# Ntropy86/review-recommender

Measured on AMD Instinct MI355X. Metric: queries/sec at top-k=100 (hybrid alpha=0.5), higher is better.
Workload: dtype f32; 1 GPU; hybrid BM25+dense alpha=0.5 top-k=100 pool=150, 10000000 products x 384 fp32, BM25 ~40 tokens/doc vocab 200000 (327073593 postings on rank 0, 11164874 postings per query), batches of 256 queries; query_sets=4, docs=10000000, docs_per_gpu=10000000, batch=256, k=100, pool=150, parallelism=single GPU: no collective

## Files before the change

include/rr_hip.h:

```cpp
#ifndef RR_HIP_H
#define RR_HIP_H

#include <stdint.h>

#ifdef __cplusplus
extern "C" {
#endif

#define RR_OK            0
#define RR_E_INVALID    -1
#define RR_E_HIP        -2
#define RR_E_NOMEM      -3
#define RR_E_STATE      -4

#define RR_DTYPE_F32     0
#define RR_DTYPE_BF16    1

#define RR_MAX_POOL   2048
#define RR_MAX_BATCH  1024
#define RR_MAX_QTERMS   64

typedef struct rr_index rr_index;
typedef struct rr_bm25  rr_bm25;

// ... 79 lines not shown
    int32_t cand_per_rank;
    int32_t bm25_f64;
    int64_t cand_rank_stride_bytes;
} rr_fuse_params;

int rr_fuse_topk_dev(rr_index* ix, const rr_fuse_params* p, int32_t n_queries,
                     const int64_t* d_rows, const float* d_dense, const float* d_bm25,
                     const double* d_n_reviews, const double* d_avg_stars, const double* d_log1p_n,
                     const float* d_rerank, const float* d_best, const float* d_gate,
                     int64_t* d_out_rows, double* d_out_cols, int32_t* d_out_order, void* stream);
int rr_fuse_topk(rr_index* ix, const rr_fuse_params* p, int32_t n_queries,
                 const int64_t* h_rows, const float* h_dense, const float* h_bm25,
                 const double* h_n_reviews, const double* h_avg_stars, const double* h_log1p_n,
                 const float* h_rerank, const float* h_best, const float* h_gate,
                 int64_t* h_out_rows, double* h_out_cols, int32_t* h_out_order);
int rr_index_gather_meta_dev(rr_index* ix, const int64_t* d_rows, int64_t n,
                             double* d_n_reviews, double* d_avg_stars, double* d_log1p_n,
                             void* stream);

#define RR_COPY_MAX_SEGS 4
typedef struct rr_copy_seg {
    void* dst;
    const void* src;
    int64_t row_bytes, rows, dst_pitch, src_pitch;
} rr_copy_seg;
int rr_copy_segments_dev(const rr_copy_seg* segs, int32_t n_segs, int32_t device, void* stream);


typedef struct rr_reviews rr_reviews;
int rr_reviews_create(const float* h_emb, int64_t n_reviews, int32_t dim, int64_t n_products,
// ... 81 lines not shown
```

review-recommender_amd/_lib.py:

```python
from __future__ import annotations

import ctypes as C
import os
import threading

from .build import DEBUG_BUILD_ID, BUILD_ID, DEBUG_LIB_PATH, LIB_PATH, library_digest

c_i32, c_i64, c_f32, c_f64, c_vp = C.c_int32, C.c_int64, C.c_float, C.c_double, C.c_void_p
P = C.POINTER


class CopySeg(C.Structure):
    _fields_ = [("dst", C.c_void_p), ("src", C.c_void_p), ("row_bytes", C.c_int64), ("rows", C.c_int64),
                ("dst_pitch", C.c_int64), ("src_pitch", C.c_int64)]


class FuseParams(C.Structure):
    _fields_ = [("w_dense", c_f64), ("w_bm25", c_f64), ("w_rerank", c_f64),
                ("w_prior", c_f64), ("w_best", c_f64), ("prior_C", c_f64),
                ("min_reviews", c_i32), ("trust_sat", c_i32), ("apply_trust", c_i32),
                ("rerank_active", c_i32), ("rerank_k", c_i32), ("k", c_i32),
                ("n_candidates", c_i32), ("pool", c_i32), ("cand_per_rank", c_i32),
                ("bm25_f64", c_i32), ("cand_rank_stride_bytes", c_i64)]

# ... 38 lines not shown
    "rr_bm25_create": (C.c_int, [c_i32, c_i64, c_i64, c_i64, c_vp, c_vp, c_vp, c_vp, c_vp,
                                 c_vp, c_vp, c_vp, c_f64, c_f64, c_f64, c_i64, P(c_vp)]),
    "rr_bm25_create_dev": (C.c_int, [c_i32, c_i64, c_i64, c_i64, c_vp, c_vp, c_vp, c_vp, c_vp,
                                     c_vp, c_vp, c_vp, c_f64, c_f64, c_f64, c_i64, P(c_vp)]),
    "rr_bm25_destroy": (C.c_int, [c_vp]),
    "rr_bm25_get_scores": (C.c_int, [c_vp, c_vp, c_i32, c_vp]),
    "rr_bm25_scores_at": (C.c_int, [c_vp, c_vp, c_vp, c_i32, c_vp, c_i32, c_i32, c_vp]),
    "rr_bm25_scores_at_dev": (C.c_int, [c_vp, c_vp, c_vp, c_i32, c_vp, c_i32, c_i32, c_vp, c_vp]),
    "rr_bm25_build": (C.c_int, [c_i32, c_i32, c_vp, c_i64, c_vp, c_i64, c_i64, c_vp, c_i64, c_i64, c_i64,
                                c_f64, c_f64, c_i64, c_vp, P(c_vp)]),
    "rr_bm25_build_stats": (C.c_int, [c_vp, c_vp, c_vp]),
    "rr_bm25_set_idf": (C.c_int, [c_vp, c_vp, c_f64]),
    "rr_bm25_copy_csr": (C.c_int, [c_vp] + [c_vp] * 7),
    "rr_fuse_topk_dev": (C.c_int, [c_vp, P(FuseParams), c_i32] + [c_vp] * 9 + [c_vp] * 3 + [c_vp]),
    "rr_fuse_topk": (C.c_int, [c_vp, P(FuseParams), c_i32] + [c_vp] * 9 + [c_vp] * 3),
    "rr_index_gather_meta_dev": (C.c_int, [c_vp, c_vp, c_i64, c_vp, c_vp, c_vp, c_vp]),
    "rr_copy_segments_dev": (C.c_int, [c_vp, c_i32, c_i32, c_vp]),
    "rr_index_matrix_changed": (C.c_int, [c_vp]),
    "rr_reviews_create": (C.c_int, [c_vp, c_i64, c_i32, c_i64, c_vp, c_vp, c_i32, c_f32, P(c_vp)]),
    "rr_reviews_destroy": (C.c_int, [c_vp]),
    "rr_reviews_best_dev": (C.c_int, [c_vp, c_vp, c_i32, c_vp, c_i32, c_i64, c_i32, c_vp, c_vp, c_vp]),
    "rr_reviews_best_cut_dev": (C.c_int, [c_vp, c_vp, c_i32, c_vp, c_i32, c_i64, c_i64, c_vp, c_vp, c_vp]),
    "rr_ce_create": (C.c_int, [c_i32, P(CEConfig), P(c_vp), c_i32, P(c_vp)]),
    "rr_ce_destroy": (C.c_int, [c_vp]),
    "rr_ce_forward_dev": (C.c_int, [c_vp, c_vp, c_vp, c_vp, c_vp, c_i32, c_i64, c_i32, c_i32, c_vp, c_vp]),
    "rr_ce_last_forward_ms": (C.c_int, [c_vp, P(c_f32)]),
    "rr_ce_range_status": (C.c_int, [c_vp, P(C.c_int32)]),
    "rr_ce_set_wide_range": (C.c_int, [c_vp, C.c_int32]),
    "rr_wp_create": (C.c_int, [c_i32, c_vp, c_vp, c_i32, c_i32, c_i32, c_i32, c_i32, P(c_vp)]),
    "rr_wp_create_utf8": (C.c_int, [c_i32, c_vp, c_vp, c_i32, c_i32, c_i32, c_i32, c_i32, c_vp, c_i32, c_vp, c_i32, c_vp, c_i32,
# ... 85 lines not shown
```

review-recommender_amd/csrc/rr_bm25.hip:

```cpp
#include "rr_common.h"

#define RR_SLICE 4096
#define RR_AT_CANDS 64

struct rr_bm25_view {
    const int64_t* post_indptr;
    const int32_t* post_docs;
    const int32_t* post_tf;
    const int64_t* doc_indptr;
    const int32_t* doc_terms;
    const int32_t* doc_tf;
    const int32_t* doc_len;
    const double* idf;
    double avgdl, k1, b;
    int64_t n_docs, n_terms, row_offset;
};

__device__ __forceinline__ double rr_bm25_term(double idf, int tf, int dl, double avgdl, double k1,
                                               double b) {
    const double f = (double)tf;
    const double one_minus_b = 1.0 - b;
    const double norm = one_minus_b + (b * (double)dl) / avgdl;
    return idf * ((f * (k1 + 1.0)) / (f + k1 * norm));
}

__device__ __forceinline__ int64_t rr_lower_bound(const int32_t* __restrict__ a, int64_t lo,
                                                  int64_t hi, int32_t key) {
    while (lo < hi) {
        const int64_t mid = lo + ((hi - lo) >> 1);
        if (a[mid] < key) lo = mid + 1; else hi = mid;
    }
    return lo;
}

__device__ __forceinline__ int64_t rr_lower_bound_wave(const int32_t* __restrict__ a, int64_t lo, int64_t hi, int32_t key) {
    const int lane = threadIdx.x & 63;
    while (hi - lo > 64) {
        const int64_t stride = (hi - lo + 63) >> 6;
        const int64_t at = lo + lane * stride;
        const bool below = at < hi && a[at] < key;
        const int c = __popcll(__ballot(below));
        if (c == 0) return lo;
        const int64_t nlo = lo + (int64_t)(c - 1) * stride + 1, nhi = lo + (int64_t)c * stride;
        lo = nlo;
        hi = nhi < hi ? nhi : hi;
    }
    const bool below = lo + lane < hi && a[lo + lane] < key;
    return lo + __popcll(__ballot(below));
// ... 46 lines not shown
                    const int32_t dd = v.post_docs[p];
                    acc[dd - d0] += rr_bm25_term(idf, v.post_tf[p], v.doc_len[dd], v.avgdl, v.k1, v.b);
                }
            }
            __syncthreads();
        }
    }
    __syncthreads();
    const bool write = touched || dirty[blockIdx.x];
    if (write)
        for (int64_t i = tid; i < d1 - d0; i += 256) out[d0 + i] = acc[i];
    if (tid == 0) dirty[blockIdx.x] = (unsigned char)touched;
}

template <int MODE>
__global__ __launch_bounds__(256) void rr_bm25_at(rr_bm25_view v, const int32_t* __restrict__ term_ids,
                                                  const int32_t* __restrict__ term_off,
                                                  const int64_t* __restrict__ rows, int pool,
                                                  float* __restrict__ out) {
    __shared__ double contrib[RR_AT_CANDS][RR_MAX_QTERMS + 1];
    const int tid = threadIdx.x;
    const int q = blockIdx.y;
    const int c0 = blockIdx.x * RR_AT_CANDS;
    const int t0 = term_off[q];
    const int nt = term_off[q + 1] - t0;
    const int nc = pool - c0 < RR_AT_CANDS ? pool - c0 : RR_AT_CANDS;
    double sum = 0.0;

    for (int jb = 0; jb < nt; jb += RR_MAX_QTERMS) {
        const int nj = nt - jb < RR_MAX_QTERMS ? nt - jb : RR_MAX_QTERMS;
        for (int i = tid; i < nc * nj; i += 256) {
            const int c = i / nj, j = i % nj;
            const int64_t d = rows[(int64_t)q * pool + c0 + c] - v.row_offset;
            const int32_t t = term_ids[t0 + jb + j];
            double val = 0.0;
            if (d >= 0 && d < v.n_docs && t >= 0 && t < v.n_terms) {
                int tf = 0;
                if (MODE == 0) {
                    const int64_t s = v.doc_indptr[d], e = v.doc_indptr[d + 1];
                    const int64_t p = rr_lower_bound(v.doc_terms, s, e, t);
                    if (p < e && v.doc_terms[p] == t) tf = v.doc_tf[p];
                } else {
                    const int64_t s = v.post_indptr[t], e = v.post_indptr[t + 1];
                    const int64_t p = rr_lower_bound(v.post_docs, s, e, (int32_t)d);
                    if (p < e && v.post_docs[p] == (int32_t)d) tf = v.post_tf[p];
                }
                if (tf > 0) val = rr_bm25_term(v.idf[t], tf, v.doc_len[d], v.avgdl, v.k1, v.b);
            }
            contrib[c][j] = val;
        }
        __syncthreads();
        if (tid < nc)
            for (int j = 0; j < nj; ++j) sum += contrib[tid][j];
        __syncthreads();
    }
    if (tid < nc) out[(int64_t)q * pool + c0 + tid] = (float)sum;
}

template <typename T>
static int rr_upload(T** dst, const T* src, size_t n) {
    *dst = nullptr;
    RR_HIP_TRY(hipMalloc((void**)dst, sizeof(T) * (n ? n : 1)));
    if (n) RR_HIP_TRY(hipMemcpy(*dst, src, sizeof(T) * n, hipMemcpyHostToDevice));
    return RR_OK;
}

static rr_bm25_view rr_view(const rr_bm25* bm) {
    rr_bm25_view v;
    v.post_indptr = bm->d_post_indptr; v.post_docs = bm->d_post_docs; v.post_tf = bm->d_post_tf;
    v.doc_indptr = bm->d_doc_indptr; v.doc_terms = bm->d_doc_terms; v.doc_tf = bm->d_doc_tf;
    v.doc_len = bm->d_doc_len; v.idf = bm->d_idf;
    v.avgdl = bm->avgdl; v.k1 = bm->k1; v.b = bm->b;
    v.n_docs = bm->n_docs; v.n_terms = bm->n_terms; v.row_offset = bm->row_offset;
    return v;
}

extern "C" int rr_bm25_create(int32_t device, int64_t n_docs, int64_t n_terms, int64_t nnz,
                              const int64_t* post_indptr, const int32_t* post_docs,
                              const int32_t* post_tf, const int64_t* doc_indptr,
                              const int32_t* doc_terms, const int32_t* doc_tf,
                              const int32_t* doc_len, const double* idf, double avgdl, double k1,
                              double b, int64_t row_offset, rr_bm25** out) {
    RR_REQUIRE(out, "rr_bm25_create: NULL out");
    *out = nullptr;
    RR_REQUIRE(n_docs >= 1 && n_docs < (1ll << 31), "rr_bm25_create: n_docs %lld out of range",
               (long long)n_docs);
    RR_REQUIRE(n_terms >= 0 && n_terms < (1ll << 31) && nnz >= 0, "rr_bm25_create: bad sizes");
    RR_REQUIRE(post_indptr && doc_indptr && doc_len && (nnz == 0 || (post_docs && post_tf && doc_terms && doc_tf)) &&
                   (n_terms == 0 || idf),
// ... 181 lines not shown
```

review-recommender_amd/csrc/rr_fuse.hip:

```cpp
#include "rr_common.h"

#define RR_FUSE_THREADS 256
#define RR_FUSE_MAXCAND RR_MAX_CANDIDATES

struct rr_fuse_dev_params {
    rr_fuse_params p;
    double log1p_sat;
    float w_dense32, w_bm2532, w_rerank32, w_best32;
    int64_t row_offset, n_rows;
    int32_t key_cap, col_cap;
};

__device__ double rr_np_pairwise(const double* a, int n) {
    if (n < 8) {
        double r = 0.0;
        for (int i = 0; i < n; ++i) r += a[i];
        return r;
    }
    if (n <= 128) {
        double r0 = a[0], r1 = a[1], r2 = a[2], r3 = a[3], r4 = a[4], r5 = a[5], r6 = a[6], r7 = a[7];
        int i;
        for (i = 8; i < n - (n % 8); i += 8) {
            r0 += a[i + 0]; r1 += a[i + 1]; r2 += a[i + 2]; r3 += a[i + 3];
            r4 += a[i + 4]; r5 += a[i + 5]; r6 += a[i + 6]; r7 += a[i + 7];
// ... 86 lines not shown
    for (int size = 2; size <= n; size <<= 1) {
        for (int stride = size >> 1; stride > 0; stride >>= 1) {
            __syncthreads();
            for (int i = threadIdx.x; i < (n >> 1); i += RR_FUSE_THREADS) {
                const int lo = 2 * i - (i & (stride - 1));
                const int hi = lo + stride;
                const bool desc = ((lo & size) == 0);
                const uint64_t a = keys[lo], b = keys[hi];
                if ((a < b) == desc) { keys[lo] = b; keys[hi] = a; }
            }
        }
    }
    __syncthreads();
}

__global__ __launch_bounds__(RR_FUSE_THREADS) void rr_fuse(
    rr_fuse_dev_params fp, const int64_t* __restrict__ g_rows, const float* __restrict__ g_dense,
    const float* __restrict__ g_bm25, const double* __restrict__ g_n, const double* __restrict__ g_avg,
    const double* __restrict__ g_l1p, const float* __restrict__ g_rerank, const float* __restrict__ g_best,
    const float* __restrict__ g_gate, const double* __restrict__ ix_n, const double* __restrict__ ix_avg,
    const double* __restrict__ ix_l1p, int64_t* __restrict__ out_rows, double* __restrict__ out_cols,
    int32_t* __restrict__ out_order) {
    extern __shared__ __align__(16) unsigned char lds[];
    const int tid = threadIdx.x;
    const int q = blockIdx.x;
    const int ncand = fp.p.n_candidates;
    const int pool = fp.p.pool;
    const int k = fp.p.k;

    const int KC = fp.key_cap, PC = fp.col_cap;
    uint64_t* keys = reinterpret_cast<uint64_t*>(lds);
    double* red = reinterpret_cast<double*>(keys + KC);
    double* c_n = red + 3 * RR_FUSE_THREADS;
    double* c_avg = c_n + PC;
    double* c_l1p = c_avg + PC;
    double* c_prior = c_l1p + PC;
    float* c_dense = reinterpret_cast<float*>(c_prior + PC);
    float* c_bm25 = c_dense + PC;
    float* c_rr = c_bm25 + PC;
    float* c_best = c_rr + PC;
// ... 55 lines not shown
                if (place < pool) c_src[place] = i;
            }
        } else {
            rr_bitonic_desc_kv(keys, slot, n_sort);
            for (int i = tid; i < pool; i += RR_FUSE_THREADS) c_src[i] = slot[i];
        }
    } else {
        for (int i = tid; i < pool; i += RR_FUSE_THREADS) c_src[i] = i;
    }
    __syncthreads();

    for (int i = tid; i < pool; i += RR_FUSE_THREADS) {
        const int s = c_src[i];
        const int64_t row = at.get(g_rows, s);
        c_dense[i] = at.get(g_dense, s);
        c_bm25[i] = g_bm25 ? at.get(g_bm25, s) : 0.f;
        c_rr[i] = (g_rerank && fp.p.rerank_active && i < fp.p.rerank_k) ? g_rerank[(int64_t)q * pool + i] : 0.f;
        c_best[i] = g_best ? g_best[(int64_t)q * pool + i] : 0.f;
        if (g_n) {
            c_n[i] = at.get(g_n, s); c_avg[i] = at.get(g_avg, s); c_l1p[i] = at.get(g_l1p, s);
        } else {
            const int64_t local = row - fp.row_offset;
            const bool ok = local >= 0 && local < fp.n_rows;
            c_n[i] = ok ? ix_n[local] : 0.0;
            c_avg[i] = ok ? ix_avg[local] : (double)NAN;
            c_l1p[i] = ok ? ix_l1p[local] : 0.0;
        }
        out_rows[(int64_t)q * pool + i] = row;
    }
    __syncthreads();

// ... 80 lines not shown
        int n_sort = 1;
        while (n_sort < pool) n_sort <<= 1;
        for (int i = tid; i < n_sort; i += RR_FUSE_THREADS) {
            uint64_t key = 0;
            if (i < pool) {
                const float f = c_final[i] + 0.0f;
                const uint32_t fk = (f == f) ? rr_f2key(f) : 0u;
                key = ((uint64_t)fk << 32) | (uint64_t)(0xFFFFFFFFu - (uint32_t)i);
            }
            keys[i] = key;
        }
        rr_bitonic_desc_pairs(keys, n_sort);
        for (int i = tid; i < k; i += RR_FUSE_THREADS)
            out_order[(int64_t)q * k + i] = (int32_t)(0xFFFFFFFFu - (uint32_t)(keys[i] & 0xFFFFFFFFu));
    }
}

__global__ void rr_gather_meta(const int64_t* __restrict__ rows, int64_t n, int64_t row_offset,
                               int64_t n_rows, const double* __restrict__ ix_n,
                               const double* __restrict__ ix_avg, const double* __restrict__ ix_l1p,
                               double* __restrict__ o_n, double* __restrict__ o_avg,
                               double* __restrict__ o_l1p) {
    const int64_t i = (int64_t)blockIdx.x * blockDim.x + threadIdx.x;
    if (i >= n) return;
    const int64_t local = rows[i] - row_offset;
    const bool ok = local >= 0 && local < n_rows;
    o_n[i] = ok ? ix_n[local] : 0.0;
    o_avg[i] = ok ? ix_avg[local] : (double)NAN;
    o_l1p[i] = ok ? ix_l1p[local] : 0.0;
}
// ... 24 lines not shown
    RR_REQUIRE(p->cand_per_rank >= 0 && p->cand_rank_stride_bytes >= 0 && p->cand_rank_stride_bytes % 8 == 0,
               "rr_fuse_topk: bad shard payload geometry");
    RR_REQUIRE(p->cand_per_rank == 0 || p->n_candidates % p->cand_per_rank == 0,
               "rr_fuse_topk: n_candidates %d is not a multiple of cand_per_rank %d", p->n_candidates, p->cand_per_rank);
    if (!n) {
        if (!ix->has_meta) {
            rr_set_error("rr_fuse_topk: index has no metadata (call rr_index_set_meta) and none was passed");
            return RR_E_STATE;
        }
        RR_REQUIRE(p->n_candidates == p->pool,
                   "rr_fuse_topk: merging shards (n_candidates > pool) needs the meta columns in the payload");
    }
    return RR_OK;
}

extern "C" int rr_fuse_topk_dev(rr_index* ix, const rr_fuse_params* p, int32_t n_queries,
                                const int64_t* d_rows, const float* d_dense, const float* d_bm25,
                                const double* d_n_reviews, const double* d_avg_stars,
                                const double* d_log1p_n, const float* d_rerank, const float* d_best,
                                const float* d_gate, int64_t* d_out_rows, double* d_out_cols,
                                int32_t* d_out_order, void* stream) {
    int rc = rr_fuse_check(ix, p, n_queries, d_rows, d_dense, d_n_reviews, d_avg_stars, d_log1p_n);
    if (rc) return rc;
    RR_REQUIRE(d_out_rows && d_out_cols && d_out_order, "rr_fuse_topk_dev: NULL output");
    RR_HIP_TRY(hipSetDevice(ix->device));
    hipStream_t st = (hipStream_t)stream;
    rr_fuse_dev_params fp;
    fp.p = *p;
    const int sat = p->trust_sat > 1 ? p->trust_sat : 1;
    fp.log1p_sat = log1p((double)sat);
    fp.w_dense32 = (float)p->w_dense;
    fp.w_bm2532 = (float)p->w_bm25;
    fp.w_rerank32 = (float)p->w_rerank;
    fp.w_best32 = (float)p->w_best;
    fp.row_offset = ix->row_offset;
    fp.n_rows = ix->n_rows;
    rr_fuse_caps(p, &fp.key_cap, &fp.col_cap);
    const size_t lds = rr_fuse_lds_bytes(fp.key_cap, fp.col_cap);
    static std::mutex attr_mu;
    static bool attr_done[64] = {false};
    {
        std::lock_guard<std::mutex> lk(attr_mu);
        if (ix->device >= 0 && ix->device < 64 && !attr_done[ix->device]) {
            RR_HIP_TRY(hipFuncSetAttribute((const void*)rr_fuse, hipFuncAttributeMaxDynamicSharedMemorySize,
                                           (int)rr_fuse_lds_bytes(RR_FUSE_MAXCAND, RR_MAX_POOL)));
            attr_done[ix->device] = true;
        }
    }
    hipLaunchKernelGGL(rr_fuse, dim3(n_queries), dim3(RR_FUSE_THREADS), lds, st, fp, d_rows, d_dense,
                       d_bm25, d_n_reviews, d_avg_stars, d_log1p_n, d_rerank, d_best, d_gate,
                       ix->d_n_reviews, ix->d_avg_stars, ix->d_log1p_n, d_out_rows, d_out_cols,
                       d_out_order);
    RR_HIP_TRY(hipGetLastError());
    return RR_OK;
}

namespace {
struct DevBuf {
    void* p = nullptr;
    hipError_t put(const void* h, size_t bytes, hipStream_t st) {
        if (!h) return hipSuccess;
        hipError_t e = hipMalloc(&p, bytes ? bytes : 1);
        if (e == hipSuccess && bytes) e = hipMemcpyAsync(p, h, bytes, hipMemcpyHostToDevice, st);
        return e;
    }
    hipError_t alloc(size_t bytes) { return hipMalloc(&p, bytes ? bytes : 1); }
    ~DevBuf() { if (p) hipFree(p); }
// ... 58 lines not shown
```

review-recommender_amd/engine.py:

```python
from __future__ import annotations

import ctypes as C
import os
import threading
from dataclasses import dataclass
from typing import Callable, Dict, List, Optional, Sequence, Tuple

import numpy as np
import pandas as pd

from . import _lib, text
from .bm25 import BM25Corpus, BM25Index, build_bm25_index_ids, factorize_corpus
from .index import MAX_POOL, ProductIndex

APP_POOL_FLOOR = 150
CLI_POOL_FLOOR = 100
APP_TRUST_SAT = 80
COLUMN_NAMES = ("_dense", "_bm25", "_prior", "_rerank", "_best", "_gate", "_trust", "_final")
_FLOAT32_COLUMNS = {"_dense", "_bm25", "_best", "_gate", "_trust", "_final"}


@dataclass
class FusionWeights:
    w_dense: float = 0.55
# ... 22 lines not shown

    def topk_rows(self) -> np.ndarray:
        return np.take_along_axis(self.pool_rows, self.order.astype(np.int64), axis=1)

    def topk_column(self, name: str) -> np.ndarray:
        c = self.columns[:, COLUMN_NAMES.index(name), :]
        return np.take_along_axis(c, self.order.astype(np.int64), axis=1)


def _torch():
    import torch
    return torch


_KERNEL_COPIES = os.environ.get("RR_NO_KERNEL_COPY") is None


class StagedTerms:
    __slots__ = ("ids", "off", "slot", "n_ids")

    def __init__(self, ids, off, slot, n_ids):
        self.ids, self.off, self.slot, self.n_ids = ids, off, slot, int(n_ids)


class StagedBatch:
    __slots__ = ("q", "terms", "ready", "slot")

    def __init__(self, q, terms, ready, slot):
        self.q, self.terms, self.ready, self.slot = q, terms, ready, slot

# ... 113 lines not shown
            (len(term_id_lists[0]) == 0) if flat_form else not any(len(t) for t in term_id_lists)
        if self.bm25 is None or empty:
            if out is None:
                return torch.zeros((B, pool), dtype=torch.float32, device=self.device)
            out.zero_()
            return out
        if out is None:
            out = torch.empty((B, pool), dtype=torch.float32, device=self.device)
        ids_dev, off_dev = (term_id_lists.ids, term_id_lists.off) if staged else self._stage_terms(term_id_lists)[:2]
        _lib.check(self.lib.rr_bm25_scores_at_dev(
            self.bm25.handle, C.c_void_p(ids_dev.data_ptr()), C.c_void_p(off_dev.data_ptr()), B,
            C.c_void_p(rows_dev.data_ptr()), pool, {"forward": 0, "postings": 1}[mode],
            C.c_void_p(out.data_ptr()), self._stream()), "rr_bm25_scores_at_dev")
        return out

    def _stage_terms(self, term_id_lists):
        torch = _torch()
        if isinstance(term_id_lists, tuple) and len(term_id_lists) == 2 and isinstance(term_id_lists[1], np.ndarray):
            flat = np.ascontiguousarray(term_id_lists[0], dtype=np.int32).reshape(-1)
            off = np.ascontiguousarray(term_id_lists[1], dtype=np.int32).reshape(-1)
        else:
            B = len(term_id_lists)
            off = np.zeros(B + 1, dtype=np.int32)
            np.cumsum([len(t) for t in term_id_lists], out=off[1:])
            flat = (np.concatenate([np.asarray(t, dtype=np.int32).reshape(-1) for t in term_id_lists])
                    if off[-1] else np.zeros(0, dtype=np.int32))
        n_off, n_ids = off.shape[0], flat.shape[0]
        need = n_off + max(n_ids, 1)
        with self._ring_lock:
            return self._stage_terms_locked(off, flat, n_off, n_ids, need)

    def _stage_terms_locked(self, off, flat, n_off, n_ids, need):
        torch = _torch()
        slot = self._stage_slots[self._stage_next % len(self._stage_slots)]
        self._stage_next += 1
        if slot["host"] is None or slot["host"].numel() < need:
            cap = max(2 * need, 16384)
            torch.cuda.synchronize(self.device)
            for sl in self._stage_slots:
                if sl["host"] is None or sl["host"].numel() < need:
                    if sl["event"] is not None:
                        sl["event"].synchronize()
                    sl["host"] = torch.empty(cap, dtype=torch.int32).pin_memory()
                    sl["dev"] = torch.empty(cap, dtype=torch.int32, device=self.device)
                    sl["event"] = torch.cuda.Event()
        else:
            slot["event"].synchronize()
        h = slot["host"].numpy()
        h[:n_off] = off
        h[n_off:n_off + n_ids] = flat
        cur = torch.cuda.current_stream(self.device)
        if slot["consumed"] is not None:
            cur.wait_event(slot["consumed"])
            slot["consumed"] = None
        if _KERNEL_COPIES:
            self.copy_segments([(slot["dev"][:need], slot["host"][:need])])
        else:
            slot["dev"][:need].copy_(slot["host"][:need], non_blocking=True)
        slot["event"].record(cur)
        return slot["dev"][n_off:n_off + max(n_ids, 1)], slot["dev"][:n_off], slot, n_ids

    def stage_batch(self, q_host, term_id_lists=None) -> "StagedBatch":
        torch = _torch()
        with self._ring_lock:
            return self._stage_batch_locked(q_host, term_id_lists)
# ... 31 lines not shown
    def fuse(self, params: "_lib.FuseParams", B: int, rows, dense, bm25, meta=None,
             rerank=None, best=None, gate=None):
        torch = _torch()
        pool, k = params.pool, params.k
        out_rows = torch.empty((B, pool), dtype=torch.int64, device=self.device)
        cols = torch.empty((B, 8, pool), dtype=torch.float64, device=self.device)
        order = torch.empty((B, k), dtype=torch.int32, device=self.device)
        p = lambda t: C.c_void_p(t.data_ptr()) if t is not None else None
        n, avg, l1p = meta if meta is not None else (None, None, None)
        _lib.check(self.lib.rr_fuse_topk_dev(
            self.index.handle, C.byref(params), B, p(rows), p(dense), p(bm25), p(n), p(avg), p(l1p),
            p(rerank), p(best), p(gate), p(out_rows), p(cols), p(order), self._stream()),
            "rr_fuse_topk_dev")
        return out_rows, cols, order

    @staticmethod
    def make_params(w: FusionWeights, k: int, pool: int, n_candidates: int, rerank_k: int,
                    cand_per_rank: int = 0, stride_bytes: int = 0, bm25_f64: bool = False) -> "_lib.FuseParams":
        return _lib.FuseParams(
            w_dense=w.w_dense, w_bm25=w.w_bm25, w_rerank=w.w_rerank, w_prior=w.w_prior,
            w_best=w.w_best, prior_C=w.prior_C, min_reviews=int(w.min_reviews),
            trust_sat=int(w.trust_sat), apply_trust=int(bool(w.apply_trust)),
            rerank_active=int(rerank_k > 0), rerank_k=int(rerank_k), k=int(k),
            n_candidates=int(n_candidates), pool=int(pool), cand_per_rank=int(cand_per_rank),
            bm25_f64=int(bool(bm25_f64)), cand_rank_stride_bytes=int(stride_bytes))

    def search_batch(self, qvecs: np.ndarray, term_id_lists: Optional[Sequence[Sequence[int]]],
                     k: int, rerank_k: int = 0, weights: Optional[FusionWeights] = None,
                     pool_floor: int = APP_POOL_FLOOR,
                     gate_fn: Optional[Callable[[np.ndarray], np.ndarray]] = None,
# ... 5 lines not shown
        q = np.ascontiguousarray(qvecs, dtype=np.float32)
        if q.ndim != 2 or q.shape[1] != self.index.dim:
            raise ValueError(f"qvecs must be (B, {self.index.dim}); got {q.shape}")
        B = q.shape[0]
        if k < 1:
            raise ValueError("k must be >= 1")
        pool = min(max(k, rerank_k, pool_floor), self.index.n_rows)
        if pool > MAX_POOL:
            raise ValueError(f"pool {pool} exceeds the kernels' limit {MAX_POOL}")
        k_eff = min(k, pool)
        rr_k = min(rerank_k, pool)
        with torch.cuda.device(self.device):
            q_dev = torch.from_numpy(q).to(self.device)
            rows, dense = self.dense_pool(q_dev, pool)
            tl = term_id_lists if term_id_lists is not None else [[] for _ in range(B)]
            bm = self.bm25_at(tl, rows, bm25_mode)
            gate = rerank = best = None
            best_ids = None
            rows_h = None
            if reviews is not None:
                best = torch.empty((B, pool), dtype=torch.float32, device=self.device)
                best_ids = torch.empty((B, pool), dtype=torch.int32, device=self.device)
                _lib.check(self.lib.rr_reviews_best_cut_dev(
                    reviews.handle, C.c_void_p(q_dev.data_ptr()), B, C.c_void_p(rows.data_ptr()), pool,
                    self.index.row_offset, int(max_scan), C.c_void_p(best.data_ptr()),
                    C.c_void_p(best_ids.data_ptr()), self._stream()), "rr_reviews_best_cut_dev")
            if gate_fn is not None or (rerank_fn is not None and rr_k > 0):
                rows_h = rows.cpu().numpy() if rows_h is None else rows_h
                if gate_fn is not None:
                    g = np.ascontiguousarray(gate_fn(rows_h), dtype=np.float32)
                    gate = torch.from_numpy(g).to(self.device)
                if rerank_fn is not None and rr_k > 0:
                    r = np.zeros((B, pool), dtype=np.float32)
                    r[:, :rr_k] = np.asarray(rerank_fn(rows_h[:, :rr_k]), dtype=np.float32)
                    rerank = torch.from_numpy(r).to(self.device)
            params = self.make_params(w, k_eff, pool, pool, rr_k, bm25_f64=bm25_f64 and self.bm25 is None)
            out_rows, cols, order = self.fuse(params, B, rows, dense, None if params.bm25_f64 else bm, None,
                                              rerank, best, gate)
            res = BatchResult(out_rows.cpu().numpy(), cols.cpu().numpy(), order.cpu().numpy(),
                              dense.cpu().numpy(), bm.cpu().numpy(), pool, k_eff)
            if best_ids is not None:
                res.best_ids, res.best_raw = best_ids.cpu().numpy(), best.cpu().numpy()
        return res


class SearchEngine:

    def __init__(self, meta: pd.DataFrame, embeddings: np.ndarray, bm25_blob: Optional[dict] = None,
                 *, encoder=None, cross_encoder=None, device: int = 0, normalize: bool = True,
                 flavour: str = "app", dtype: str = "f32", reviews: Optional[Tuple] = None,
                 bm25_build: str = "device", index: Optional[ProductIndex] = None):
        if flavour not in ("app", "cli"):
            raise ValueError("flavour must be 'app' or 'cli'")
# ... 196 lines not shown
```

review-recommender_amd/sharded.py:

```python
from __future__ import annotations

import ctypes as C
import os
from dataclasses import dataclass
from typing import Optional, Sequence, Tuple

import numpy as np

from . import _lib
from .engine import FusionWeights, HybridSearcher
from .index import MAX_CANDIDATES


def shard_bounds(n_rows: int, world: int, rank: int) -> Tuple[int, int]:
    if not (0 <= rank < world):
        raise ValueError("rank outside [0, world)")
    base, extra = divmod(n_rows, world)
    lo = rank * base + min(rank, extra)
    return lo, lo + base + (1 if rank < extra else 0)


@dataclass(frozen=True)
class PayloadLayout:
    n_queries: int
# ... 266 lines not shown
        import torch
        w = weights or FusionWeights()
        B = q_dev.shape[0]
        pool = min(max(k, rerank_k, pool_floor), self.n_total)
        self._check_merge_size(pool)
        pool_local = min(pool, self.s.index.n_rows)
        rr_k = min(rerank_k, pool)
        if self.world > 1:
            assert pool_local == pool, "each shard needs at least `pool` rows"
        tl = term_id_lists if term_id_lists is not None else [[] for _ in range(B)]
        s = self.s
        two_pass = gate_fn is not None or (rerank_fn is not None and rr_k > 0)
        if self.world == 1 and not self.force_payload:
            self._flush_overlap()
            rows, dense = s.dense_pool(q_dev, pool)
            bm = s.bm25_at(tl, rows, bm25_mode)
            gate = rerank = None
            if two_pass:
                gate, rerank = self._pool_columns(rows, B, pool, rr_k, gate_fn, rerank_fn)
            return s.fuse(HybridSearcher.make_params(w, min(k, pool), pool, pool, rr_k), B, rows, dense, bm,
                          None, rerank, None, gate)
        return self.finish(self.submit(q_dev, term_id_lists, k, weights, pool_floor, bm25_mode, rerank_k, gate_fn, rerank_fn))

    def submit(self, q_dev, term_id_lists, k: int, weights: Optional[FusionWeights] = None, pool_floor: int = 150,
               bm25_mode: str = "forward", rerank_k: int = 0, gate_fn=None, rerank_fn=None) -> "PendingBatch":
        w = weights or FusionWeights()
        B = q_dev.shape[0]
        pool = min(max(k, rerank_k, pool_floor), self.n_total)
        self._check_merge_size(pool)
        pool_local = min(pool, self.s.index.n_rows)
# ... 174 lines not shown
```

Baseline: 133,400 queries/s.

## Fuse BM25 candidate scoring into the fusion top-k kernel

Adds a single kernel that computes BM25 scores for each query's candidate pool straight into LDS and then runs the fusion/top-k body, so the separate bm25_at launch and its global round trip go away. It also shares a batched binary-search helper that interleaves R independent lookups per thread to hide memory latency, and lets term staging pass host-pinned buffers in place. The fused path uses one block per query (256 blocks for a batch), which lowers parallelism for the scoring phase compared with the old grid over candidate tiles.

```diff
diff --git a/include/rr_hip.h b/include/rr_hip.h
--- a/include/rr_hip.h
+++ b/include/rr_hip.h
@@ -117,6 +117,11 @@
                  const double* h_n_reviews, const double* h_avg_stars, const double* h_log1p_n,
                  const float* h_rerank, const float* h_best, const float* h_gate,
                  int64_t* h_out_rows, double* h_out_cols, int32_t* h_out_order);
+#define RR_BM25_FUSE_MAX_POOL 512
+int rr_bm25_fuse(rr_index* ix, rr_bm25* bm, const rr_fuse_params* p, int32_t n_queries,
+                 const int32_t* d_term_ids, const int32_t* d_term_off, int32_t mode,
+                 const int64_t* d_rows, const float* d_dense, const float* d_best, float* d_out_bm25,
+                 int64_t* d_out_rows, double* d_out_cols, int32_t* d_out_order, void* stream);
 int rr_index_gather_meta_dev(rr_index* ix, const int64_t* d_rows, int64_t n,
                              double* d_n_reviews, double* d_avg_stars, double* d_log1p_n,
                              void* stream);
diff --git a/review-recommender_amd/_lib.py b/review-recommender_amd/_lib.py
--- a/review-recommender_amd/_lib.py
+++ b/review-recommender_amd/_lib.py
@@ -76,6 +76,7 @@
     "rr_bm25_copy_csr": (C.c_int, [c_vp] + [c_vp] * 7),
     "rr_fuse_topk_dev": (C.c_int, [c_vp, P(FuseParams), c_i32] + [c_vp] * 9 + [c_vp] * 3 + [c_vp]),
     "rr_fuse_topk": (C.c_int, [c_vp, P(FuseParams), c_i32] + [c_vp] * 9 + [c_vp] * 3),
+    "rr_bm25_fuse": (C.c_int, [c_vp, c_vp, P(FuseParams), c_i32, c_vp, c_vp, c_i32] + [c_vp] * 4 + [c_vp] * 3 + [c_vp]),
     "rr_index_gather_meta_dev": (C.c_int, [c_vp, c_vp, c_i64, c_vp, c_vp, c_vp, c_vp]),
     "rr_copy_segments_dev": (C.c_int, [c_vp, c_i32, c_i32, c_vp]),
     "rr_index_matrix_changed": (C.c_int, [c_vp]),
diff --git a/review-recommender_amd/csrc/rr_bm25.hip b/review-recommender_amd/csrc/rr_bm25.hip
--- a/review-recommender_amd/csrc/rr_bm25.hip
+++ b/review-recommender_amd/csrc/rr_bm25.hip
@@ -1,37 +1,7 @@
-#include "rr_common.h"
+#include "rr_bm25_dev.h"
 
 #define RR_SLICE 4096
 #define RR_AT_CANDS 64
-
-struct rr_bm25_view {
-    const int64_t* post_indptr;
-    const int32_t* post_docs;
-    const int32_t* post_tf;
-    const int64_t* doc_indptr;
-    const int32_t* doc_terms;
-    const int32_t* doc_tf;
-    const int32_t* doc_len;
-    const double* idf;
-    double avgdl, k1, b;
-    int64_t n_docs, n_terms, row_offset;
-};
-
-__device__ __forceinline__ double rr_bm25_term(double idf, int tf, int dl, double avgdl, double k1,
-                                               double b) {
-    const double f = (double)tf;
-    const double one_minus_b = 1.0 - b;
-    const double norm = one_minus_b + (b * (double)dl) / avgdl;
-    return idf * ((f * (k1 + 1.0)) / (f + k1 * norm));
-}
-
-__device__ __forceinline__ int64_t rr_lower_bound(const int32_t* __restrict__ a, int64_t lo,
-                                                  int64_t hi, int32_t key) {
-    while (lo < hi) {
-        const int64_t mid = lo + ((hi - lo) >> 1);
-        if (a[mid] < key) lo = mid + 1; else hi = mid;
-    }
-    return lo;
-}
 
 __device__ __forceinline__ int64_t rr_lower_bound_wave(const int32_t* __restrict__ a, int64_t lo, int64_t hi, int32_t key) {
     const int lane = threadIdx.x & 63;
@@ -108,46 +78,19 @@
 }
 
 template <int MODE>
-__global__ __launch_bounds__(256) void rr_bm25_at(rr_bm25_view v, const int32_t* __restrict__ term_ids,
-                                                  const int32_t* __restrict__ term_off,
-                                                  const int64_t* __restrict__ rows, int pool,
-                                                  float* __restrict__ out) {
-    __shared__ double contrib[RR_AT_CANDS][RR_MAX_QTERMS + 1];
+__global__ __launch_bounds__(RR_AT_THREADS) void rr_bm25_at(rr_bm25_view v, const int32_t* __restrict__ term_ids,
+                                                            const int32_t* __restrict__ term_off,
+                                                            const int64_t* __restrict__ rows, int pool,
+                                                            float* __restrict__ out) {
+    __shared__ double contrib[RR_AT_CANDS * (RR_MAX_QTERMS + 1)];
     const int tid = threadIdx.x;
     const int q = blockIdx.y;
     const int c0 = blockIdx.x * RR_AT_CANDS;
     const int t0 = term_off[q];
     const int nt = term_off[q + 1] - t0;
     const int nc = pool - c0 < RR_AT_CANDS ? pool - c0 : RR_AT_CANDS;
-    double sum = 0.0;
-
-    for (int jb = 0; jb < nt; jb += RR_MAX_QTERMS) {
-        const int nj = nt - jb < RR_MAX_QTERMS ? nt - jb : RR_MAX_QTERMS;
-        for (int i = tid; i < nc * nj; i += 256) {
-            const int c = i / nj, j = i % nj;
-            const int64_t d = rows[(int64_t)q * pool + c0 + c] - v.row_offset;
-            const int32_t t = term_ids[t0 + jb + j];
-            double val = 0.0;
-            if (d >= 0 && d < v.n_docs && t >= 0 && t < v.n_terms) {
-                int tf = 0;
-                if (MODE == 0) {
-                    const int64_t s = v.doc_indptr[d], e = v.doc_indptr[d + 1];
-                    const int64_t p = rr_lower_bound(v.doc_terms, s, e, t);
-                    if (p < e && v.doc_terms[p] == t) tf = v.doc_tf[p];
-                } else {
-                    const int64_t s = v.post_indptr[t], e = v.post_indptr[t + 1];
-                    const int64_t p = rr_lower_bound(v.post_docs, s, e, (int32_t)d);
-                    if (p < e && v.post_docs[p] == (int32_t)d) tf = v.post_tf[p];
-                }
-                if (tf > 0) val = rr_bm25_term(v.idf[t], tf, v.doc_len[d], v.avgdl, v.k1, v.b);
-            }
-            contrib[c][j] = val;
-        }
-        __syncthreads();
-        if (tid < nc)
-            for (int j = 0; j < nj; ++j) sum += contrib[tid][j];
-        __syncthreads();
-    }
+    const double sum = rr_bm25_at_rows<MODE, 1>(v, term_ids, t0, nt, rows + (int64_t)q * pool + c0, nc, RR_MAX_QTERMS, contrib,
+                                                RR_MAX_QTERMS + 1);
     if (tid < nc) out[(int64_t)q * pool + c0 + tid] = (float)sum;
 }
 
@@ -157,16 +100,6 @@
     RR_HIP_TRY(hipMalloc((void**)dst, sizeof(T) * (n ? n : 1)));
     if (n) RR_HIP_TRY(hipMemcpy(*dst, src, sizeof(T) * n, hipMemcpyHostToDevice));
     return RR_OK;
-}
-
-static rr_bm25_view rr_view(const rr_bm25* bm) {
-    rr_bm25_view v;
-    v.post_indptr = bm->d_post_indptr; v.post_docs = bm->d_post_docs; v.post_tf = bm->d_post_tf;
-    v.doc_indptr = bm->d_doc_indptr; v.doc_terms = bm->d_doc_terms; v.doc_tf = bm->d_doc_tf;
-    v.doc_len = bm->d_doc_len; v.idf = bm->d_idf;
-    v.avgdl = bm->avgdl; v.k1 = bm->k1; v.b = bm->b;
-    v.n_docs = bm->n_docs; v.n_terms = bm->n_terms; v.row_offset = bm->row_offset;
-    return v;
 }
 
 extern "C" int rr_bm25_create(int32_t device, int64_t n_docs, int64_t n_terms, int64_t nnz,
diff --git a/review-recommender_amd/csrc/rr_bm25_dev.h b/review-recommender_amd/csrc/rr_bm25_dev.h
--- /dev/null
+++ b/review-recommender_amd/csrc/rr_bm25_dev.h
@@ -0,0 +1,121 @@
+#pragma once
+#include "rr_common.h"
+
+struct rr_bm25_view {
+    const int64_t* post_indptr;
+    const int32_t* post_docs;
+    const int32_t* post_tf;
+    const int64_t* doc_indptr;
+    const int32_t* doc_terms;
+    const int32_t* doc_tf;
+    const int32_t* doc_len;
+    const double* idf;
+    double avgdl, k1, b;
+    int64_t n_docs, n_terms, row_offset;
+};
+
+static inline rr_bm25_view rr_view(const rr_bm25* bm) {
+    rr_bm25_view v;
+    v.post_indptr = bm->d_post_indptr; v.post_docs = bm->d_post_docs; v.post_tf = bm->d_post_tf;
+    v.doc_indptr = bm->d_doc_indptr; v.doc_terms = bm->d_doc_terms; v.doc_tf = bm->d_doc_tf;
+    v.doc_len = bm->d_doc_len; v.idf = bm->d_idf;
+    v.avgdl = bm->avgdl; v.k1 = bm->k1; v.b = bm->b;
+    v.n_docs = bm->n_docs; v.n_terms = bm->n_terms; v.row_offset = bm->row_offset;
+    return v;
+}
+
+#ifdef __HIPCC__
+#define RR_AT_THREADS 256
+
+__device__ __forceinline__ double rr_bm25_term(double idf, int tf, int dl, double avgdl, double k1,
+                                               double b) {
+    const double f = (double)tf;
+    const double one_minus_b = 1.0 - b;
+    const double norm = one_minus_b + (b * (double)dl) / avgdl;
+    return idf * ((f * (k1 + 1.0)) / (f + k1 * norm));
+}
+
+template <int MODE, int R>
+__device__ __forceinline__ void rr_bm25_at_contrib(const rr_bm25_view& v, const int32_t* __restrict__ tq,
+                                                   const int64_t* __restrict__ rows_c, int nc, int nj,
+                                                   double* __restrict__ contrib, int ld) {
+    const int n = nc * nj;
+    const int32_t* __restrict__ list = MODE == 0 ? v.doc_terms : v.post_docs;
+    const int32_t* __restrict__ list_tf = MODE == 0 ? v.doc_tf : v.post_tf;
+    for (int i0 = threadIdx.x; i0 < n; i0 += RR_AT_THREADS * R) {
+        int64_t lo[R], hi[R], end[R];
+        int32_t key[R], dl[R];
+        double idf[R];
+        bool ok[R];
+#pragma unroll
+        for (int r = 0; r < R; ++r) {
+            const int i = i0 + RR_AT_THREADS * r;
+            const bool live = i < n;
+            const int64_t d = rows_c[live ? i / nj : 0] - v.row_offset;
+            const int32_t t = tq[live ? i % nj : 0];
+            ok[r] = live && d >= 0 && d < v.n_docs && t >= 0 && t < v.n_terms;
+            lo[r] = hi[r] = end[r] = 0;
+            key[r] = 0; dl[r] = 0; idf[r] = 0.0;
+            if (ok[r]) {
+                const int64_t* __restrict__ ip = MODE == 0 ? v.doc_indptr + d : v.post_indptr + t;
+                lo[r] = ip[0];
+                hi[r] = end[r] = ip[1];
+                key[r] = MODE == 0 ? t : (int32_t)d;
+                dl[r] = v.doc_len[d];
+                idf[r] = v.idf[t];
+            }
+        }
+        bool more = true;
+        while (more) {
+            int64_t mid[R];
+            int32_t x[R];
+#pragma unroll
+            for (int r = 0; r < R; ++r) {
+                mid[r] = lo[r] + ((hi[r] - lo[r]) >> 1);
+                x[r] = list[lo[r] < hi[r] ? mid[r] : 0];
+            }
+            more = false;
+#pragma unroll
+            for (int r = 0; r < R; ++r) {
+                if (lo[r] < hi[r]) {
+                    if (x[r] < key[r]) lo[r] = mid[r] + 1; else hi[r] = mid[r];
+                }
+                more = more || lo[r] < hi[r];
+            }
+        }
+        bool found[R];
+        int32_t tf[R];
+#pragma unroll
+        for (int r = 0; r < R; ++r) {
+            const bool in = ok[r] && lo[r] < end[r];
+            found[r] = in && list[in ? lo[r] : 0] == key[r];
+        }
+#pragma unroll
+        for (int r = 0; r < R; ++r) tf[r] = list_tf[found[r] ? lo[r] : 0];
+#pragma unroll
+        for (int r = 0; r < R; ++r) {
+            const int i = i0 + RR_AT_THREADS * r;
+            double val = 0.0;
+            if (found[r] && tf[r] > 0) val = rr_bm25_term(idf[r], tf[r], dl[r], v.avgdl, v.k1, v.b);
+            if (i < n) contrib[(i / nj) * ld + i % nj] = val;
+        }
+    }
+}
+
+template <int MODE, int R>
+__device__ __forceinline__ double rr_bm25_at_rows(const rr_bm25_view& v, const int32_t* __restrict__ term_ids, int t0, int nt,
+                                                  const int64_t* __restrict__ rows_c, int nc, int qt,
+                                                  double* __restrict__ contrib, int ld) {
+    const int tid = threadIdx.x;
+    double sum = 0.0;
+    for (int jb = 0; jb < nt; jb += qt) {
+        const int nj = nt - jb < qt ? nt - jb : qt;
+        rr_bm25_at_contrib<MODE, R>(v, term_ids + t0 + jb, rows_c, nc, nj, contrib, ld);
+        __syncthreads();
+        if (tid < nc)
+            for (int j = 0; j < nj; ++j) sum += contrib[tid * ld + j];
+        __syncthreads();
+    }
+    return sum;
+}
+#endif
diff --git a/review-recommender_amd/csrc/rr_fuse.hip b/review-recommender_amd/csrc/rr_fuse.hip
--- a/review-recommender_amd/csrc/rr_fuse.hip
+++ b/review-recommender_amd/csrc/rr_fuse.hip
@@ -1,4 +1,5 @@
 #include "rr_common.h"
+#include "rr_bm25_dev.h"
 
 #define RR_FUSE_THREADS 256
 #define RR_FUSE_MAXCAND RR_MAX_CANDIDATES
@@ -124,16 +125,20 @@
     __syncthreads();
 }
 
-__global__ __launch_bounds__(RR_FUSE_THREADS) void rr_fuse(
-    rr_fuse_dev_params fp, const int64_t* __restrict__ g_rows, const float* __restrict__ g_dense,
-    const float* __restrict__ g_bm25, const double* __restrict__ g_n, const double* __restrict__ g_avg,
-    const double* __restrict__ g_l1p, const float* __restrict__ g_rerank, const float* __restrict__ g_best,
-    const float* __restrict__ g_gate, const double* __restrict__ ix_n, const double* __restrict__ ix_avg,
-    const double* __restrict__ ix_l1p, int64_t* __restrict__ out_rows, double* __restrict__ out_cols,
-    int32_t* __restrict__ out_order) {
-    extern __shared__ __align__(16) unsigned char lds[];
+__device__ __forceinline__ float* rr_fuse_bm25_column(unsigned char* lds, int key_cap, int col_cap) {
+    double* red = reinterpret_cast<double*>(reinterpret_cast<uint64_t*>(lds) + key_cap);
+    return reinterpret_cast<float*>(red + 3 * RR_FUSE_THREADS + 4 * col_cap) + col_cap;
+}
+
+template <bool BM25_IN_LDS>
+__device__ __forceinline__ void rr_fuse_body(
+    const rr_fuse_dev_params& fp, const int q, unsigned char* lds, const int64_t* __restrict__ g_rows,
+    const float* __restrict__ g_dense, const float* __restrict__ g_bm25, const double* __restrict__ g_n,
+    const double* __restrict__ g_avg, const double* __restrict__ g_l1p, const float* __restrict__ g_rerank,
+    const float* __restrict__ g_best, const float* __restrict__ g_gate, const double* __restrict__ ix_n,
+    const double* __restrict__ ix_avg, const double* __restrict__ ix_l1p, int64_t* __restrict__ out_rows,
+    double* __restrict__ out_cols, int32_t* __restrict__ out_order) {
     const int tid = threadIdx.x;
-    const int q = blockIdx.x;
     const int ncand = fp.p.n_candidates;
     const int pool = fp.p.pool;
     const int k = fp.p.k;
@@ -219,7 +224,7 @@
         const int s = c_src[i];
         const int64_t row = at.get(g_rows, s);
         c_dense[i] = at.get(g_dense, s);
-        c_bm25[i] = g_bm25 ? at.get(g_bm25, s) : 0.f;
+        if (!BM25_IN_LDS) c_bm25[i] = g_bm25 ? at.get(g_bm25, s) : 0.f;
         c_rr[i] = (g_rerank && fp.p.rerank_active && i < fp.p.rerank_k) ? g_rerank[(int64_t)q * pool + i] : 0.f;
         c_best[i] = g_best ? g_best[(int64_t)q * pool + i] : 0.f;
         if (g_n) {
@@ -330,6 +335,50 @@
         for (int i = tid; i < k; i += RR_FUSE_THREADS)
             out_order[(int64_t)q * k + i] = (int32_t)(0xFFFFFFFFu - (uint32_t)(keys[i] & 0xFFFFFFFFu));
     }
+}
+
+__global__ __launch_bounds__(RR_FUSE_THREADS) void rr_fuse(
+    rr_fuse_dev_params fp, const int64_t* __restrict__ g_rows, const float* __restrict__ g_dense,
+    const float* __restrict__ g_bm25, const double* __restrict__ g_n, const double* __restrict__ g_avg,
+    const double* __restrict__ g_l1p, const float* __restrict__ g_rerank, const float* __restrict__ g_best,
+    const float* __restrict__ g_gate, const double* __restrict__ ix_n, const double* __restrict__ ix_avg,
+    const double* __restrict__ ix_l1p, int64_t* __restrict__ out_rows, double* __restrict__ out_cols,
+    int32_t* __restrict__ out_order) {
+    extern __shared__ __align__(16) unsigned char lds[];
+    rr_fuse_body<false>(fp, blockIdx.x, lds, g_rows, g_dense, g_bm25, g_n, g_avg, g_l1p, g_rerank, g_best, g_gate, ix_n, ix_avg,
+                        ix_l1p, out_rows, out_cols, out_order);
+}
+
+#define RR_BF_QTERMS 16
+#define RR_BF_LD (RR_BF_QTERMS + 1)
+template <int MODE>
+__global__ __launch_bounds__(RR_FUSE_THREADS) void rr_bm25_fuse_k(
+    rr_fuse_dev_params fp, rr_bm25_view v, const int32_t* __restrict__ term_ids, const int32_t* __restrict__ term_off,
+    const int64_t* __restrict__ g_rows, const float* __restrict__ g_dense, const float* __restrict__ g_best,
+    const double* __restrict__ ix_n, const double* __restrict__ ix_avg, const double* __restrict__ ix_l1p,
+    float* __restrict__ out_bm25, int64_t* __restrict__ out_rows, double* __restrict__ out_cols,
+    int32_t* __restrict__ out_order, int contrib_off) {
+    extern __shared__ __align__(16) unsigned char lds[];
+    const int tid = threadIdx.x;
+    const int q = blockIdx.x;
+    const int pool = fp.p.pool;
+    float* c_bm25 = rr_fuse_bm25_column(lds, fp.key_cap, fp.col_cap);
+    double* contrib = reinterpret_cast<double*>(lds + contrib_off);
+    const int t0 = term_off[q];
+    const int nt = term_off[q + 1] - t0;
+    for (int c0 = 0; c0 < pool; c0 += RR_FUSE_THREADS) {
+        const int nc = pool - c0 < RR_FUSE_THREADS ? pool - c0 : RR_FUSE_THREADS;
+        const double sum = rr_bm25_at_rows<MODE, 4>(v, term_ids, t0, nt, g_rows + (int64_t)q * pool + c0, nc, RR_BF_QTERMS,
+                                                    contrib, RR_BF_LD);
+        if (tid < nc) {
+            const float s = (float)sum;
+            c_bm25[c0 + tid] = s;
+            if (out_bm25) out_bm25[(int64_t)q * pool + c0 + tid] = s;
+        }
+    }
+    __syncthreads();
+    rr_fuse_body<true>(fp, q, lds, g_rows, g_dense, nullptr, nullptr, nullptr, nullptr, nullptr, g_best, nullptr, ix_n, ix_avg,
+                       ix_l1p, out_rows, out_cols, out_order);
 }
 
 __global__ void rr_gather_meta(const int64_t* __restrict__ rows, int64_t n, int64_t row_offset,
@@ -384,6 +433,21 @@
     return RR_OK;
 }
 
+static rr_fuse_dev_params rr_fuse_dev_params_of(const rr_index* ix, const rr_fuse_params* p) {
+    rr_fuse_dev_params fp;
+    fp.p = *p;
+    const int sat = p->trust_sat > 1 ? p->trust_sat : 1;
+    fp.log1p_sat = log1p((double)sat);
+    fp.w_dense32 = (float)p->w_dense;
+    fp.w_bm2532 = (float)p->w_bm25;
+    fp.w_rerank32 = (float)p->w_rerank;
+    fp.w_best32 = (float)p->w_best;
+    fp.row_offset = ix->row_offset;
+    fp.n_rows = ix->n_rows;
+    rr_fuse_caps(p, &fp.key_cap, &fp.col_cap);
+    return fp;
+}
+
 extern "C" int rr_fuse_topk_dev(rr_index* ix, const rr_fuse_params* p, int32_t n_queries,
                                 const int64_t* d_rows, const float* d_dense, const float* d_bm25,
                                 const double* d_n_reviews, const double* d_avg_stars,
@@ -395,17 +459,7 @@
     RR_REQUIRE(d_out_rows && d_out_cols && d_out_order, "rr_fuse_topk_dev: NULL output");
     RR_HIP_TRY(hipSetDevice(ix->device));
     hipStream_t st = (hipStream_t)stream;
-    rr_fuse_dev_params fp;
-    fp.p = *p;
-    const int sat = p->trust_sat > 1 ? p->trust_sat : 1;
-    fp.log1p_sat = log1p((double)sat);
-    fp.w_dense32 = (float)p->w_dense;
-    fp.w_bm2532 = (float)p->w_bm25;
-    fp.w_rerank32 = (float)p->w_rerank;
-    fp.w_best32 = (float)p->w_best;
-    fp.row_offset = ix->row_offset;
-    fp.n_rows = ix->n_rows;
-    rr_fuse_caps(p, &fp.key_cap, &fp.col_cap);
+    const rr_fuse_dev_params fp = rr_fuse_dev_params_of(ix, p);
     const size_t lds = rr_fuse_lds_bytes(fp.key_cap, fp.col_cap);
     static std::mutex attr_mu;
     static bool attr_done[64] = {false};
@@ -421,6 +475,51 @@
                        d_bm25, d_n_reviews, d_avg_stars, d_log1p_n, d_rerank, d_best, d_gate,
                        ix->d_n_reviews, ix->d_avg_stars, ix->d_log1p_n, d_out_rows, d_out_cols,
                        d_out_order);
+    RR_HIP_TRY(hipGetLastError());
+    return RR_OK;
+}
+
+static size_t rr_bm25_fuse_lds_bytes(int key_cap, int col_cap) {
+    return rr_fuse_lds_bytes(key_cap, col_cap) + sizeof(double) * RR_FUSE_THREADS * RR_BF_LD;
+}
+
+extern "C" int rr_bm25_fuse(rr_index* ix, rr_bm25* bm, const rr_fuse_params* p, int32_t n_queries,
+                            const int32_t* d_term_ids, const int32_t* d_term_off, int32_t mode,
+                            const int64_t* d_rows, const float* d_dense, const float* d_best, float* d_out_bm25,
+                            int64_t* d_out_rows, double* d_out_cols, int32_t* d_out_order, void* stream) {
+    int rc = rr_fuse_check(ix, p, n_queries, d_rows, d_dense, nullptr, nullptr, nullptr);
+    if (rc) return rc;
+    RR_REQUIRE(bm && d_term_ids && d_term_off && d_out_rows && d_out_cols && d_out_order, "rr_bm25_fuse: NULL argument");
+    RR_REQUIRE(mode == 0 || mode == 1, "rr_bm25_fuse: mode must be 0 (forward) or 1 (postings)");
+    RR_REQUIRE(p->pool <= RR_BM25_FUSE_MAX_POOL, "rr_bm25_fuse: pool %d above %d (use rr_bm25_scores_at_dev + rr_fuse_topk_dev)",
+               p->pool, RR_BM25_FUSE_MAX_POOL);
+    RR_REQUIRE(p->cand_per_rank == 0 && !p->rerank_active && !p->bm25_f64,
+               "rr_bm25_fuse: shard payloads, a reranker and the float64 zeros column take the two separate calls");
+    RR_REQUIRE(bm->device == ix->device, "rr_bm25_fuse: index on device %d, BM25 on device %d", ix->device, bm->device);
+    if (!bm->d_idf) { rr_set_error("rr_bm25_fuse: no idf yet (rr_bm25_set_idf)"); return RR_E_STATE; }
+    RR_HIP_TRY(hipSetDevice(ix->device));
+    hipStream_t st = (hipStream_t)stream;
+    const rr_fuse_dev_params fp = rr_fuse_dev_params_of(ix, p);
+    const size_t k3 = rr_fuse_lds_bytes(fp.key_cap, fp.col_cap), lds = rr_bm25_fuse_lds_bytes(fp.key_cap, fp.col_cap);
+    static std::mutex attr_mu;
+    static bool attr_done[64] = {false};
+    {
+        std::lock_guard<std::mutex> lk(attr_mu);
+        if (ix->device >= 0 && ix->device < 64 && !attr_done[ix->device]) {
+            const int most = (int)rr_bm25_fuse_lds_bytes(RR_BM25_FUSE_MAX_POOL, RR_BM25_FUSE_MAX_POOL);
+            RR_HIP_TRY(hipFuncSetAttribute((const void*)rr_bm25_fuse_k<0>, hipFuncAttributeMaxDynamicSharedMemorySize, most));
+            RR_HIP_TRY(hipFuncSetAttribute((const void*)rr_bm25_fuse_k<1>, hipFuncAttributeMaxDynamicSharedMemorySize, most));
+            attr_done[ix->device] = true;
+        }
+    }
+    if (mode == 0)
+        hipLaunchKernelGGL((rr_bm25_fuse_k<0>), dim3(n_queries), dim3(RR_FUSE_THREADS), lds, st, fp, rr_view(bm), d_term_ids,
+                           d_term_off, d_rows, d_dense, d_best, ix->d_n_reviews, ix->d_avg_stars, ix->d_log1p_n, d_out_bm25,
+                           d_out_rows, d_out_cols, d_out_order, (int)k3);
+    else
+        hipLaunchKernelGGL((rr_bm25_fuse_k<1>), dim3(n_queries), dim3(RR_FUSE_THREADS), lds, st, fp, rr_view(bm), d_term_ids,
+                           d_term_off, d_rows, d_dense, d_best, ix->d_n_reviews, ix->d_avg_stars, ix->d_log1p_n, d_out_bm25,
+                           d_out_rows, d_out_cols, d_out_order, (int)k3);
     RR_HIP_TRY(hipGetLastError());
     return RR_OK;
 }
diff --git a/review-recommender_amd/engine.py b/review-recommender_amd/engine.py
--- a/review-recommender_amd/engine.py
+++ b/review-recommender_amd/engine.py
@@ -60,6 +60,8 @@
 
 
 _KERNEL_COPIES = os.environ.get("RR_NO_KERNEL_COPY") is None
+_TAIL_LEGACY = os.environ.get("RR_TAIL_LEGACY") is not None
+BM25_FUSE_MAX_POOL = 512
 
 
 class StagedTerms:
@@ -203,7 +205,7 @@
             C.c_void_p(out.data_ptr()), self._stream()), "rr_bm25_scores_at_dev")
         return out
 
-    def _stage_terms(self, term_id_lists):
+    def _stage_terms(self, term_id_lists, in_place: bool = False):
         torch = _torch()
         if isinstance(term_id_lists, tuple) and len(term_id_lists) == 2 and isinstance(term_id_lists[1], np.ndarray):
             flat = np.ascontiguousarray(term_id_lists[0], dtype=np.int32).reshape(-1)
@@ -217,9 +219,9 @@
         n_off, n_ids = off.shape[0], flat.shape[0]
         need = n_off + max(n_ids, 1)
         with self._ring_lock:
-            return self._stage_terms_locked(off, flat, n_off, n_ids, need)
-
-    def _stage_terms_locked(self, off, flat, n_off, n_ids, need):
+            return self._stage_terms_locked(off, flat, n_off, n_ids, need, in_place)
+
+    def _stage_terms_locked(self, off, flat, n_off, n_ids, need, in_place=False):
         torch = _torch()
         slot = self._stage_slots[self._stage_next % len(self._stage_slots)]
         self._stage_next += 1
@@ -238,6 +240,8 @@
         h = slot["host"].numpy()
         h[:n_off] = off
         h[n_off:n_off + n_ids] = flat
+        if in_place:
+            return slot["host"][n_off:n_off + max(n_ids, 1)], slot["host"][:n_off], slot, n_ids
         cur = torch.cuda.current_stream(self.device)
         if slot["consumed"] is not None:
             cur.wait_event(slot["consumed"])
@@ -299,6 +303,35 @@
             "rr_fuse_topk_dev")
         return out_rows, cols, order
 
+    def can_bm25_fuse(self, term_id_lists, pool: int) -> bool:
+        if _TAIL_LEGACY or self.bm25 is None or pool > BM25_FUSE_MAX_POOL:
+            return False
+        if isinstance(term_id_lists, StagedTerms):
+            return term_id_lists.n_ids > 0
+        if isinstance(term_id_lists, tuple) and len(term_id_lists) == 2 and isinstance(term_id_lists[1], np.ndarray):
+            return len(term_id_lists[0]) > 0
+        return any(len(t) for t in term_id_lists)
+
+    def bm25_fuse(self, params: "_lib.FuseParams", B: int, term_id_lists, rows, dense, mode: str = "forward", best=None,
+                  bm25_out=None):
+        torch = _torch()
+        pool, k = params.pool, params.k
+        out_rows = torch.empty((B, pool), dtype=torch.int64, device=self.device)
+        cols = torch.empty((B, 8, pool), dtype=torch.float64, device=self.device)
+        order = torch.empty((B, k), dtype=torch.int32, device=self.device)
+        p = lambda t: C.c_void_p(t.data_ptr()) if t is not None else None
+        slot = None
+        if isinstance(term_id_lists, StagedTerms):
+            ids, off = term_id_lists.ids, term_id_lists.off
+        else:
+            ids, off, slot, _ = self._stage_terms(term_id_lists, in_place=_KERNEL_COPIES)
+        _lib.check(self.lib.rr_bm25_fuse(
+            self.index.handle, self.bm25.handle, C.byref(params), B, p(ids), p(off), {"forward": 0, "postings": 1}[mode],
+            p(rows), p(dense), p(best), p(bm25_out), p(out_rows), p(cols), p(order), self._stream()), "rr_bm25_fuse")
+        if slot is not None and _KERNEL_COPIES:
+            slot["event"].record(torch.cuda.current_stream(self.device))
+        return out_rows, cols, order
+
     @staticmethod
     def make_params(w: FusionWeights, k: int, pool: int, n_candidates: int, rerank_k: int,
                     cand_per_rank: int = 0, stride_bytes: int = 0, bm25_f64: bool = False) -> "_lib.FuseParams":
@@ -334,7 +367,8 @@
             q_dev = torch.from_numpy(q).to(self.device)
             rows, dense = self.dense_pool(q_dev, pool)
             tl = term_id_lists if term_id_lists is not None else [[] for _ in range(B)]
-            bm = self.bm25_at(tl, rows, bm25_mode)
+            one_launch = gate_fn is None and rr_k == 0 and self.can_bm25_fuse(tl, pool)
+            bm = self.bm25_at(tl, rows, bm25_mode) if not one_launch else None
             gate = rerank = best = None
             best_ids = None
             rows_h = None
@@ -355,8 +389,12 @@
                     r[:, :rr_k] = np.asarray(rerank_fn(rows_h[:, :rr_k]), dtype=np.float32)
                     rerank = torch.from_numpy(r).to(self.device)
             params = self.make_params(w, k_eff, pool, pool, rr_k, bm25_f64=bm25_f64 and self.bm25 is None)
-            out_rows, cols, order = self.fuse(params, B, rows, dense, None if params.bm25_f64 else bm, None,
-                                              rerank, best, gate)
+            if one_launch:
+                bm = torch.empty((B, pool), dtype=torch.float32, device=self.device)
+                out_rows, cols, order = self.bm25_fuse(params, B, tl, rows, dense, bm25_mode, best, bm25_out=bm)
+            else:
+                out_rows, cols, order = self.fuse(params, B, rows, dense, None if params.bm25_f64 else bm, None,
+                                                  rerank, best, gate)
             res = BatchResult(out_rows.cpu().numpy(), cols.cpu().numpy(), order.cpu().numpy(),
                               dense.cpu().numpy(), bm.cpu().numpy(), pool, k_eff)
             if best_ids is not None:
diff --git a/review-recommender_amd/sharded.py b/review-recommender_amd/sharded.py
--- a/review-recommender_amd/sharded.py
+++ b/review-recommender_amd/sharded.py
@@ -304,6 +304,8 @@
         if self.world == 1 and not self.force_payload:
             self._flush_overlap()
             rows, dense = s.dense_pool(q_dev, pool)
+            if not two_pass and rr_k == 0 and s.can_bm25_fuse(tl, pool):
+                return s.bm25_fuse(HybridSearcher.make_params(w, min(k, pool), pool, pool, 0), B, tl, rows, dense, bm25_mode)
             bm = s.bm25_at(tl, rows, bm25_mode)
             gate = rerank = None
             if two_pass:
```

Result: no change. 133,900 queries/s (median of 3 runs) (+0.4%).
